# jaesung-cs/vulkan_radix_sort

Measured on AMD Instinct MI355X. Metric: GItems/s at N=2^25 (keys & key+value); achieved HBM GB/s vs peak, higher is better.
Workload: dtype u32

## Files before the change

vulkan_radix_sort_amd/csrc/vrdx_kernels.hip:

```cpp
#include <hip/hip_runtime.h>
#include <stdint.h>

#include <type_traits>

#include "vrdx_kernels.h"
#include "vrdx_layout.h"

namespace vrdx {



#ifdef VRDX_TRACE
#define VRDX_STAMP(slot)                                      \
  do {                                                        \
    if (a.trace != nullptr && tid == 0) stamps[slot] = wall_clock64(); \
  } while (0)
#else
#define VRDX_STAMP(slot) \
  do {                   \
  } while (0)
#endif


typedef uint32_t u32x4 __attribute__((ext_vector_type(4)));
// ... 1992 lines not shown
    lo += v[k] & 0xFFFFu;
    hi += v[k] >> 16;
  }
  if (tid < 64u) {
    const uint32_t mine = tid < 2 * WORDS ? total[tid] : 0u;
    const uint32_t inclusive = WaveInclusiveScan(mine);
    if (tid < 2 * WORDS) {
      uint32_t base = inclusive - mine;
#pragma unroll
      for (uint32_t q = 0; q < 16; ++q) base += below[q];
      a.bucketBase[firstBucket + tid] = base;
      if (topWindow) a.bucketCount[firstBucket + tid] = mine;
      if (mine > a.cap) atomicOr(a.overflowWord, kMsdDeclineBucket);
    }
  }
}

template <uint32_t BITS, bool KV>
__device__ __forceinline__ void ScatterMsdBody(const MsdArgs a) {
  constexpr int THREADS = 1024, KPT = 32, WAVES = THREADS / 64;
  constexpr uint32_t TILE = kMsdTileKeys, D = 1u << BITS, ROW = D / 2u;
  static_assert(THREADS * KPT == TILE && ROW <= (uint32_t)THREADS && WAVES * ROW <= TILE, "geometry");
  extern __shared__ __attribute__((aligned(16))) uint32_t smem[];
  uint32_t* const sorted = smem;
  uint32_t* const counters = smem;
  uint32_t* const tileOffset = smem + TILE;
  uint32_t* const scanScratch = tileOffset + D;

  const int tid = threadIdx.x;
  const int lane = tid & 63;
  const int wave = tid >> 6;
  const uint32_t n = ElementCount(a.maxCount, a.countPtr);
  const uint32_t perXcd = gridDim.x / 8u;
  const uint32_t tile = (blockIdx.x % 8u) * perXcd + blockIdx.x / 8u;
  const uint32_t slots = a.tileKeys / (uint32_t)THREADS;
  const uint32_t frame = a.tileKeys;
  const uint32_t tileStart = tile * frame;
  const uint32_t decided = *a.overflowWord;
  if ((decided & kMsdDeclineMask) != 0u) {
    if (blockIdx.x == 0 && tid == 0 && a.declinedPlans != nullptr) atomicAdd(a.declinedPlans, 1u);
    return;
  }
  const uint32_t SHIFT = (decided >> kMsdShiftShift) & kMsdShiftMask;
  if (((decided >> kMsdModeShift) & kMsdModeMask) == kMsdModeIdentical) {
    if (blockIdx.x == 0 && tid == 0) *a.planWord = kMsdVerdictSorted;
    return;
  }
  const uint32_t valid = tile < a.tiles && tileStart < n ? ((n - tileStart) < frame ? (n - tileStart) : frame) : 0u;
  const uint32_t tileEnd = tileStart + valid;
  const uint32_t loadBase = tileStart + wave * (slots * 64) + lane;
  uint32_t key[KPT];
  LoadStriped<KPT, true, true>(a.keysCaller, loadBase, tileEnd, valid == frame, 0xFFFFFFFFu, key, slots);
  uint32_t prefixWord = 0, base0 = 0, base1 = 0;
  if ((uint32_t)tid < ROW && valid != 0) {
    prefixWord = a.tileCounts[(size_t)tile * ROW + tid];
    base0 = a.bucketBase[2 * tid];
    base1 = a.bucketBase[2 * tid + 1];
  }
  if (blockIdx.x == 0 && tid == 0) *a.planWord = kMsdVerdictRuns | (SHIFT << kMsdShiftShift);
  if (valid == 0) return;

  uint32_t* const myRow = counters + wave * ROW;
#pragma unroll
  for (uint32_t i = 0; i < ROW / 256u; ++i) reinterpret_cast<u32x4*>(myRow)[lane + 64 * i] = u32x4{0u, 0u, 0u, 0u};
  uint32_t rank[KPT / 2];
  RankPacked16<KPT, true>(key, SHIFT, BITS, myRow, lane, rank, slots);
  ForgetDerivedValues<KPT>(key);
  LdsBarrier();

  uint32_t column[WAVES];
  const uint32_t totals = (uint32_t)tid < ROW ? ColumnRead<ROW, WAVES>(counters, tid, column) : 0u;
  const uint32_t count0 = totals & 0xFFFFu, count1 = totals >> 16;
  const uint32_t local0 = BlockExclusiveScanAll<THREADS>(count0 + count1, scanScratch, tid);
  const uint32_t local1 = local0 + count0;
  if ((uint32_t)tid < ROW) {
    ColumnBasesFrom<ROW, WAVES>(counters, tid, local0 | (local1 << 16), column);
    tileOffset[2 * tid] = base0 + (prefixWord & 0xFFFFu) - local0;
    tileOffset[2 * tid + 1] = base1 + (prefixWord >> 16) - local1;
  }
  LdsBarrier();
  PositionsPacked16<KPT, TILE, true>(key, SHIFT, BITS, myRow, rank, slots);
  LdsBarrier();
#pragma unroll
  for (int i = 0; i < KPT; ++i) {
    if (i % 4 == 0 && (uint32_t)i >= slots) break;
    sorted[(rank[i / 2] >> (16 * (i % 2))) & 0xFFFFu] = key[i];
  }
  LdsBarrier();
  uint32_t val[KV ? KPT : 1];
  if constexpr (KV)
    LoadStriped<KPT, true, true>(a.valuesCaller, loadBase, tileEnd, valid == frame, 0u, val, slots);

  constexpr int QUADS = KPT / 4;
  constexpr int B = 4;
  uint32_t quadDigits[KV ? QUADS : 1];
  uint32_t boundaryQuad[2] = {~0u, ~0u};
  uint32_t boundaryDigits[2][2] = {{0, 0}, {0, 0}};
  if ((uint32_t)tid < ROW) {
    if (count0 != 0 && (local0 & 3u) != 0 && local0 < valid) boundaryQuad[0] = local0 & ~3u;
    if (count1 != 0 && (local1 & 3u) != 0 && local1 < valid) boundaryQuad[1] = local1 & ~3u;
  }
  if (tid == 0 && (valid & 3u) != 0) boundaryQuad[0] = valid & ~3u;
  auto scatterQuads = [&](uint32_t* out, bool keysPhase) {
#pragma unroll
    for (int j0 = 0; j0 < QUADS; j0 += B) {
      if (4u * (uint32_t)j0 * THREADS >= valid) break;
      u32x4 w4[B];
      uint32_t o[B];
      bool whole[B];
#pragma unroll
      for (int b = 0; b < B; ++b) w4[b] = *reinterpret_cast<const u32x4*>(&sorted[4u * (tid + (j0 + b) * THREADS)]);
#pragma unroll
      for (int b = 0; b < B; ++b) {
        const int j = j0 + b;
        const uint32_t p = StagingSlot<TILE>(4u * (tid + j * THREADS));
        uint32_t d0, d3;
        if (keysPhase) {
          d0 = __builtin_amdgcn_ubfe(w4[b][0], SHIFT, BITS);
          d3 = __builtin_amdgcn_ubfe(w4[b][3], SHIFT, BITS);
          if constexpr (KV) quadDigits[j] = d0 | (d3 << 16);
        } else {
          d0 = quadDigits[KV ? j : 0] & 0xFFFFu;
          d3 = quadDigits[KV ? j : 0] >> 16;
        }
        whole[b] = p + 3 < valid && d0 == d3;
        o[b] = tileOffset[d0] + p;
        asm volatile("" : "+v"(o[b]));
      }
#pragma unroll
      for (int b = 0; b < B; ++b)
        if (whole[b]) StoreQuad(out, o[b], w4[b]);
    }
#pragma unroll
    for (int s = 0; s < 2; ++s) {
      if (boundaryQuad[s] == ~0u) continue;
      const u32x4 q = *reinterpret_cast<const u32x4*>(&sorted[StagingSlot<TILE>(boundaryQuad[s])]);
      if (keysPhase) {
        boundaryDigits[s][0] = __builtin_amdgcn_ubfe(q[0], SHIFT, BITS) | (__builtin_amdgcn_ubfe(q[1], SHIFT, BITS) << 16);
        boundaryDigits[s][1] = __builtin_amdgcn_ubfe(q[2], SHIFT, BITS) | (__builtin_amdgcn_ubfe(q[3], SHIFT, BITS) << 16);
      }
#pragma unroll
      for (int c = 0; c < 4; ++c) {
        const uint32_t d = (boundaryDigits[s][c / 2] >> (16 * (c % 2))) & 0xFFFFu;
        if (boundaryQuad[s] + c < valid) StoreWord(out, tileOffset[d] + boundaryQuad[s] + c, q[c]);
      }
    }
  };
  scatterQuads(a.keysScratch, true);
  if constexpr (KV) {
    LdsBarrier();
#pragma unroll
    for (int i = 0; i < KPT; ++i) {
      if (i % 4 == 0 && (uint32_t)i >= slots) break;
      sorted[(rank[i / 2] >> (16 * (i % 2))) & 0xFFFFu] = val[i];
    }
    LdsBarrier();
    scatterQuads(a.valuesScratch, false);
  }
}

template <uint32_t BITS>
__device__ __forceinline__ void ScatterMsdPairBody(const MsdArgs a) {
  constexpr int THREADS = 1024, KPT = 32, WAVES = THREADS / 64;
  constexpr uint32_t TILE = kMsdTileKeys, D = 1u << BITS, ROW = D / 2u;
  static_assert(2 * WAVES * ROW <= TILE, "both sub-tiles' counter rows inside the staging buffer");
  extern __shared__ __attribute__((aligned(16))) uint32_t smem[];
  uint32_t* const sorted = smem;
  uint32_t* const counters = smem;
  uint32_t* const tileOffset = smem + TILE;
  uint32_t* const scanScratch = tileOffset + D;

  const int tid = threadIdx.x;
  const int lane = tid & 63;
  const int wave = tid >> 6;
  const uint32_t n = ElementCount(a.maxCount, a.countPtr);
  const uint32_t pairs = (a.tiles + 1u) / 2u;
  const uint32_t perXcd = (pairs + 7u) / 8u;
  const uint32_t pair = (blockIdx.x % 8u) * perXcd + blockIdx.x / 8u;
  const uint32_t slots = a.tileKeys / (uint32_t)THREADS;
  const uint32_t frame = a.tileKeys;
  const uint32_t decided = *a.overflowWord;
  if ((decided & kMsdDeclineMask) != 0u) {
    if (blockIdx.x == 0 && tid == 0 && a.declinedPlans != nullptr) atomicAdd(a.declinedPlans, 1u);
    return;
  }
  const uint32_t SHIFT = (decided >> kMsdShiftShift) & kMsdShiftMask;
  if (((decided >> kMsdModeShift) & kMsdModeMask) == kMsdModeIdentical) {
    if (blockIdx.x == 0 && tid == 0) *a.planWord = kMsdVerdictSorted;
    return;
  }
  const uint32_t tileA = 2u * pair;
  const uint32_t startA = tileA * frame, startB = startA + frame;
  const bool exists = blockIdx.x < 8u * perXcd && pair < pairs && startA < n;
  const uint32_t left = exists ? n - startA : 0u;
  const uint32_t validA = left < frame ? left : frame;
  const uint32_t validB = left > frame ? (left - frame < frame ? left - frame : frame) : 0u;
  const uint32_t valid = validA + validB;
  const uint32_t baseA = startA + wave * (slots * 64) + lane, baseB = baseA + frame;
  uint32_t keyA[KPT], keyB[KPT];
  LoadStriped<KPT, true, true>(a.keysCaller, baseA, startA + validA, validA == frame, 0xFFFFFFFFu, keyA, slots);
  LoadStriped<KPT, true, true>(a.keysCaller, baseB, startB + validB, validB == frame, 0xFFFFFFFFu, keyB, slots);
  uint32_t prefixWord = 0, base0 = 0, base1 = 0;
  if ((uint32_t)tid < ROW && valid != 0) {
    prefixWord = a.tileCounts[(size_t)tileA * ROW + tid];
    base0 = a.bucketBase[2 * tid];
    base1 = a.bucketBase[2 * tid + 1];
  }
  if (blockIdx.x == 0 && tid == 0) *a.planWord = kMsdVerdictRuns | (SHIFT << kMsdShiftShift);
  if (valid == 0) return;

  uint32_t* const rowA = counters + wave * ROW;
  uint32_t* const rowB = counters + (WAVES + wave) * ROW;
#pragma unroll
  for (uint32_t i = 0; i < ROW / 256u; ++i) {
    reinterpret_cast<u32x4*>(rowA)[lane + 64 * i] = u32x4{0u, 0u, 0u, 0u};
    reinterpret_cast<u32x4*>(rowB)[lane + 64 * i] = u32x4{0u, 0u, 0u, 0u};
  }
  uint32_t posA[KPT / 2], posB[KPT / 2];
  RankPacked16<KPT, true>(keyA, SHIFT, BITS, rowA, lane, posA, slots);
  ForgetDerivedValues<KPT>(keyA);
  RankPacked16<KPT, true>(keyB, SHIFT, BITS, rowB, lane, posB, slots);
  ForgetDerivedValues<KPT>(keyB);
  LdsBarrier();

  const uint32_t totals = (uint32_t)tid < ROW ? ColumnTotals<ROW, 2 * WAVES>(counters, tid) : 0u;
  const uint32_t count0 = totals & 0xFFFFu, count1 = totals >> 16;
  const uint32_t local0 = BlockExclusiveScanAll<THREADS>(count0 + count1, scanScratch, tid);
  const uint32_t local1 = local0 + count0;
  if ((uint32_t)tid < ROW) {
    ColumnBases<ROW, 2 * WAVES>(counters, tid, local0 | (local1 << 16));
    tileOffset[2 * tid] = base0 + (prefixWord & 0xFFFFu) - local0;
    tileOffset[2 * tid + 1] = base1 + (prefixWord >> 16) - local1;
  }
  LdsBarrier();
  PositionsPacked16<KPT, TILE, true, true>(keyA, SHIFT, BITS, rowA, posA, slots);
  PositionsPacked16<KPT, TILE, true, true>(keyB, SHIFT, BITS, rowB, posB, slots);
  LdsBarrier();

  constexpr int QUADS = KPT / 4;
  constexpr int B = 2;
  uint32_t boundaryQuad[2] = {~0u, ~0u};
  if ((uint32_t)tid < ROW) {
    if (count0 != 0 && (local0 & 3u) != 0 && local0 < valid) boundaryQuad[0] = local0 & ~3u;
    if (count1 != 0 && (local1 & 3u) != 0 && local1 < valid) boundaryQuad[1] = local1 & ~3u;
  }
  if (tid == 0 && (valid & 3u) != 0) boundaryQuad[0] = valid & ~3u;
#pragma unroll 1
  for (uint32_t half = 0; half < 2; ++half) {
    const uint32_t from = half * frame;
    if (from >= valid) break;
    if (half != 0) LdsBarrier();
#pragma unroll
    for (int i = 0; i < KPT; ++i) {
      if (i % 4 == 0 && (uint32_t)i >= slots) break;
      const uint32_t pa = ((posA[i / 2] >> (16 * (i % 2))) & 0xFFFFu) - from;
      const uint32_t pb = ((posB[i / 2] >> (16 * (i % 2))) & 0xFFFFu) - from;
      if (pa < frame) sorted[StagingSlot<TILE>(pa)] = keyA[i];
      if (pb < frame) sorted[StagingSlot<TILE>(pb)] = keyB[i];
    }
    LdsBarrier();
    const uint32_t here = valid - from < frame ? valid - from : frame;
#pragma unroll
    for (int j0 = 0; j0 < QUADS; j0 += B) {
      if (4u * (uint32_t)j0 * THREADS >= here) break;
      u32x4 w4[B];
      uint32_t o[B];
      bool whole[B];
#pragma unroll
      for (int b = 0; b < B; ++b) w4[b] = *reinterpret_cast<const u32x4*>(&sorted[4u * (tid + (j0 + b) * THREADS)]);
#pragma unroll
      for (int b = 0; b < B; ++b) {
        const uint32_t p = StagingSlot<TILE>(4u * (tid + (j0 + b) * THREADS));
        const uint32_t d0 = __builtin_amdgcn_ubfe(w4[b][0], SHIFT, BITS), d3 = __builtin_amdgcn_ubfe(w4[b][3], SHIFT, BITS);
        whole[b] = p + 3 < here && d0 == d3;
        o[b] = tileOffset[d0] + from + p;
        asm volatile("" : "+v"(o[b]));
      }
#pragma unroll
      for (int b = 0; b < B; ++b)
        if (whole[b]) StoreQuad(a.keysScratch, o[b], w4[b]);
    }
#pragma unroll
    for (int s = 0; s < 2; ++s) {
      const uint32_t q0 = boundaryQuad[s] - from;
      if (boundaryQuad[s] == ~0u || q0 >= frame) continue;
      const u32x4 q = *reinterpret_cast<const u32x4*>(&sorted[StagingSlot<TILE>(q0)]);
#pragma unroll
      for (int c = 0; c < 4; ++c)
        if (q0 + c < here) StoreWord(a.keysScratch, tileOffset[__builtin_amdgcn_ubfe(q[c], SHIFT, BITS)] + boundaryQuad[s] + c, q[c]);
    }
  }
}
template <uint32_t BITS, bool KV>
constexpr bool MsdScatterTakesPairs() { return !KV && BITS == 10; }
template <uint32_t BITS, bool KV>
__device__ __forceinline__ void ScatterMsdRole(const MsdArgs a) {
  if constexpr (MsdScatterTakesPairs<BITS, KV>())
    ScatterMsdPairBody<BITS>(a);
  else
    ScatterMsdBody<BITS, KV>(a);
}


template <uint32_t BITS, int KPT, bool KV, int THREADS = 1024>
__device__ __forceinline__ void BucketSort2Bucket(const MsdArgs a, const uint32_t bucket, const uint32_t below, const bool streamOut) {
  constexpr int WAVES = THREADS / 64;
  static_assert(THREADS == 1024 || THREADS == 512, "one or two words of a counter row per thread");
  constexpr uint32_t TILE = THREADS * KPT;
  constexpr uint32_t ROW = 1024;
  static_assert(32u - BITS <= 22u, "two passes of at most eleven bits");
  static_assert(TILE <= 65536 && WAVES * ROW <= TILE && KPT % 4 == 0, "packed positions; the staging buffer covers the counters");
  extern __shared__ __attribute__((aligned(16))) uint32_t smem[];
  uint32_t* const staged = smem;
  uint32_t* const counters = smem;
  uint32_t* const scanScratch = smem + TILE;

  const int tid = threadIdx.x;
  const int lane = tid & 63;
  const int wave = tid >> 6;
  const uint32_t W0 = (below + 1u) / 2u, W1 = below / 2u;
  constexpr uint32_t passes = 2u;
  const uint32_t myBase = (uint32_t)__builtin_amdgcn_readfirstlane((int)a.bucketBase[bucket]);
  const uint32_t n = (uint32_t)__builtin_amdgcn_readfirstlane((int)a.bucketCount[bucket]);
  if (n == 0) return;
  const uint32_t* const keysIn = a.keysScratch + myBase;
  uint32_t* const keysOut = a.keysCaller + myBase;
  const uint32_t* const valuesIn = KV ? a.valuesScratch + myBase : nullptr;
  uint32_t* const valuesOut = KV ? a.valuesCaller + myBase : nullptr;

  constexpr bool DYN = true;
  const uint32_t chunks = (n + 255u) / 256u;
  const uint32_t base = chunks / WAVES, extra = chunks % WAVES;
  const uint32_t w = (uint32_t)__builtin_amdgcn_readfirstlane(wave);
  const uint32_t slots = 4u * (base + (w < extra ? 1u : 0u));
  const uint32_t first = 256u * (w * base + (w < extra ? w : extra)) + lane;
  uint32_t key[KPT];
  uint32_t val[KV ? KPT : 1];
  LoadStriped<KPT, false, DYN>(keysIn, first, n, false, 0xFFFFFFFFu, key, slots);
  if constexpr (KV) LoadStriped<KPT, false, DYN>(valuesIn, first, n, false, 0u, val, slots);

  uint32_t* const myRow = counters + wave * ROW;
#pragma unroll 1
  for (uint32_t pass = 0; pass < passes; ++pass) {
    const uint32_t shift = pass == 0 ? 0u : W0;
    const uint32_t width = pass == 0 ? W0 : W1;
    const uint32_t words = width > 1u ? 1u << (width - 1u) : 1u;
#pragma unroll
    for (uint32_t i = 0; i < ROW / 256u; ++i)
      if (256u * i < words) reinterpret_cast<u32x4*>(myRow)[lane + 64 * i] = u32x4{0u, 0u, 0u, 0u};
    uint32_t rank[KPT / 2];
    RankPacked16<KPT, DYN>(key, shift, width, myRow, lane, rank, slots);
    ForgetDerivedValues<KPT>(key);
    LdsBarrier();
    uint32_t firstNow = first;
    asm volatile("" : "+v"(firstNow));
    if constexpr (THREADS == 512) {
      const bool mine = KV || 2u * (uint32_t)tid < words;
      u32x2 column[WAVES];
      const u32x2 totals = mine ? ColumnPairRead<ROW, WAVES>(counters, tid, column) : u32x2{0u, 0u};
      const uint32_t count0 = totals[0] & 0xFFFFu, count1 = totals[0] >> 16, count2 = totals[1] & 0xFFFFu;
      const uint32_t local0 = BlockExclusiveScanAll<THREADS>(count0 + count1 + count2 + (totals[1] >> 16), scanScratch + 16 * pass, tid);
      const uint32_t local2 = local0 + count0 + count1;
      if (mine)
        ColumnPairBasesFrom<ROW, WAVES>(counters, tid, u32x2{local0 | ((local0 + count0) << 16), local2 | ((local2 + count2) << 16)}, column);
    } else if constexpr (!KV) {
      const bool mine = (uint32_t)tid < words;
      uint32_t column[WAVES];
      const uint32_t totals = mine ? ColumnRead<ROW, WAVES>(counters, tid, column) : 0u;
      const uint32_t count0 = totals & 0xFFFFu;
      const uint32_t local0 = BlockExclusiveScanAll<THREADS>(count0 + (totals >> 16), scanScratch + 16 * pass, tid);
      if (mine) ColumnBasesFrom<ROW, WAVES>(counters, tid, local0 | ((local0 + count0) << 16), column);
    } else {
      const bool mine = (uint32_t)tid < words;
      const uint32_t totals = mine ? ColumnTotals<ROW, WAVES>(counters, tid) : 0u;
      const uint32_t count0 = totals & 0xFFFFu;
      const uint32_t local0 = BlockExclusiveScanAll<THREADS>(count0 + (totals >> 16), scanScratch + 16 * pass, tid);
      if (mine) ColumnBases<ROW, WAVES>(counters, tid, local0 | ((local0 + count0) << 16));
    }
    LdsBarrier();
    PositionsPacked16<KPT, TILE, DYN>(key, shift, width, myRow, rank, slots);
    LdsBarrier();
#pragma unroll
    for (int i = 0; i < KPT; ++i) {
      if (DYN && i % 4 == 0 && (uint32_t)i >= slots) break;
      staged[(rank[i / 2] >> (16 * (i % 2))) & 0xFFFFu] = key[i];
    }
    LdsBarrier();
#pragma unroll
    for (int i = 0; i < KPT; ++i) {
      if (DYN && i % 4 == 0 && (uint32_t)i >= slots) break;
      key[i] = staged[StagingSlot<TILE>(firstNow + 64 * i)];
    }
    if constexpr (KV) {
      LdsBarrier();
#pragma unroll
      for (int i = 0; i < KPT; ++i) {
        if (DYN && i % 4 == 0 && (uint32_t)i >= slots) break;
        staged[(rank[i / 2] >> (16 * (i % 2))) & 0xFFFFu] = val[i];
      }
      LdsBarrier();
#pragma unroll
      for (int i = 0; i < KPT; ++i) {
        if (DYN && i % 4 == 0 && (uint32_t)i >= slots) break;
        val[i] = staged[StagingSlot<TILE>(firstNow + 64 * i)];
      }
    }
    LdsBarrier();
  }
  if (KV ? a.maxCount > kStreamingLoadsAbove : streamOut) {
    asm volatile("; non-temporal output" ::: "memory");
#pragma unroll
    for (int i = 0; i < KPT; ++i) {
      if (DYN && i % 4 == 0 && (uint32_t)i >= slots) break;
      const uint32_t index = first + 64 * i;
      if (index < n) {
        __builtin_nontemporal_store(key[i], &keysOut[index]);
        if constexpr (KV) __builtin_nontemporal_store(val[i], &valuesOut[index]);
      }
    }
    asm volatile("" ::: "memory");
  } else {
#pragma unroll
    for (int i = 0; i < KPT; ++i) {
      if (DYN && i % 4 == 0 && (uint32_t)i >= slots) break;
      const uint32_t index = first + 64 * i;
      if (index < n) {
        keysOut[index] = key[i];
        if constexpr (KV) valuesOut[index] = val[i];
      }
    }
  }
}

template <uint32_t BITS, int KPT, bool KV, int THREADS = 1024>
__device__ __forceinline__ void BucketSort2Body(const MsdArgs a, const uint32_t workgroups) {
  const uint32_t verdict = *a.planWord;
  if ((verdict & kMsdVerdictMask) != kMsdVerdictRuns) return;
  const uint32_t below = (verdict >> kMsdShiftShift) & kMsdShiftMask;
  uint32_t streamedBuckets = 0u;
  if constexpr (!KV && THREADS == 1024 && BITS == 10)
    if (a.maxCount > kStreamingLoadsAbove) streamedBuckets = (1u << BITS) - min(a.plainTail, 1u << BITS);
#pragma unroll 1
  for (uint32_t bucket = blockIdx.x; bucket < (1u << BITS); bucket += workgroups)
    BucketSort2Bucket<BITS, KPT, KV, THREADS>(a, bucket, below, bucket < streamedBuckets);
}

template <uint32_t BITS, bool KV>
__global__ __launch_bounds__(512, 4) void bucket_sort2_half_kernel(MsdArgs a) {
  BucketSort2Body<BITS, kMsdHalfCap / 512, KV, 512>(a, gridDim.x);
}

template <uint32_t BITS, bool KV, bool DYN>
__device__ __forceinline__ void FallbackPassBody(const OnesweepArgs p) {
  if constexpr (KV)
    OnesweepBody<1024, 32, true, true, DYN>(p);
  else
    OnesweepPairBody<1024, 32, DYN>(p);
}

template <uint32_t BITS, bool KV, bool DYN>
__global__ __launch_bounds__(1024) void msd_scatter_or_pass0_kernel(MsdArgs m, OnesweepArgs p) {
  if ((*m.overflowWord & kMsdDeclineMask) == 0u) {
    ScatterMsdRole<BITS, KV>(m);
    return;
  }
  if (blockIdx.x > p.statusRows) return;
  FallbackPassBody<BITS, KV, DYN>(p);
  if (blockIdx.x == 0 && threadIdx.x == 0 && m.declinedPlans != nullptr) atomicAdd(m.declinedPlans, 1u);
}
template <uint32_t BITS, bool KV, bool DYN>
__global__ __launch_bounds__(1024) void msd_buckets_or_pass1_kernel(MsdArgs m, OnesweepArgs p) {
  const uint32_t verdict = *m.planWord & kMsdVerdictMask;
  if (verdict < kMsdVerdictRuns) {
    if (blockIdx.x > p.statusRows) return;
    FallbackPassBody<BITS, KV, DYN>(p);
    return;
  }
  const uint32_t workgroups = min(gridDim.x, (1u << BITS) / 2u);
  if (verdict == kMsdVerdictRuns && blockIdx.x < workgroups)
    BucketSort2Body<BITS, (KV ? kMsdCapKeyValue : kMsdCapKeys) / 1024, KV>(m, workgroups);
}

__device__ __forceinline__ uint32_t OrderCheckKey(uint32_t tid, uint32_t wave, uint32_t slot) {
  uint32_t x = (blockIdx.x * 1024u + tid) * 0x9E3779B9u + slot * 0x85EBCA6Bu;
  x ^= x >> 15; x *= 0x2C1B3C6Du; x ^= x >> 12; x *= 0x297A2D39u; x ^= x >> 15;
  const uint32_t mode = (blockIdx.x + wave + slot) % 6u;
  const uint32_t mask = mode == 0 ? 0u : mode == 1 ? 1u : mode == 2 ? 3u : mode == 3 ? 15u : mode == 4 ? 0x21u : 255u;
  return x & mask;
}

__global__ __launch_bounds__(1024) void lds_order_check_kernel(uint32_t* mismatches, uint32_t* sticky) {
  __shared__ uint32_t counters[2 * 16 * 256];
  const int tid = threadIdx.x, lane = tid & 63, wave = tid >> 6;
  for (int i = tid; i < 2 * 16 * 256; i += 1024) counters[i] = 0;
  __syncthreads();
  uint32_t* const histA = counters + wave * 256;
  uint32_t* const histB = counters + (16 + wave) * 256;
  uint32_t bad = 0;
  for (uint32_t round = 0; round < 8; ++round) {
    uint32_t key[8], ra[8], rb[8];
#pragma unroll
    for (int i = 0; i < 8; ++i) key[i] = OrderCheckKey(tid, wave, round * 8 + i);
    RankAtomic<8, false>(key, 0, histA, lane, ra);
    RankBallot<8>(key, 0, histB, lane, rb);
#pragma unroll
    for (int i = 0; i < 8; ++i) bad += ra[i] != rb[i];
  }
#pragma unroll 1
  for (uint32_t form = 0; form < 2; ++form) {
    uint32_t key[32], want[16];
#pragma unroll
    for (int i = 0; i < 32; ++i) key[i] = OrderCheckKey(tid, wave, 64 + 32 * form + i);
    RankBallot<32, true>(key, 0, histB, lane, want);
    if (form == 0) {
      uint32_t ra[32];
      RankAtomic<32, false>(key, 0, histA, lane, ra);
#pragma unroll
      for (int i = 0; i < 16; ++i) bad += (ra[2 * i] | (ra[2 * i + 1] << 16)) != want[i];
    } else {
      uint32_t rp[16];
      RankAtomic<32, true>(key, 0, histA, lane, rp);
#pragma unroll
      for (int i = 0; i < 16; ++i) bad += rp[i] != want[i];
    }
  }
  if (bad != 0) {
    if (mismatches != nullptr) atomicAdd(mismatches, bad);
    if (sticky != nullptr) atomicOr(sticky, 2u);
  }
}

__device__ __forceinline__ uint32_t OrderCheckDigit11(uint32_t tid, uint32_t wave, uint32_t slot) {
  uint32_t x = (blockIdx.x * 1024u + tid) * 0x9E3779B9u + slot * 0x85EBCA6Bu + 0x7F4A7C15u;
  x ^= x >> 15; x *= 0x2C1B3C6Du; x ^= x >> 12; x *= 0x297A2D39u; x ^= x >> 15;
  const uint32_t mode = (blockIdx.x + wave + slot) % 7u;
  const uint32_t mask = mode == 0 ? 0u : mode == 1 ? 1u : mode == 2 ? 3u : mode == 3 ? 15u : mode == 4 ? 0x421u : mode == 5 ? 63u : 2047u;
  return ((x & mask) + (mode == 5 ? 0x300u : 0u)) & 2047u;
}

__global__ __launch_bounds__(1024) void lds_order_check_packed_kernel(uint32_t* mismatches, uint32_t* sticky) {
  extern __shared__ __attribute__((aligned(16))) uint32_t smem[];
  const int tid = threadIdx.x, lane = tid & 63, wave = tid >> 6;
  uint32_t* const rowA = smem + wave * 1024;
  uint32_t* const rowB = smem + (16 + wave) * 1024;
  for (int i = lane; i < 1024; i += 64) rowA[i] = rowB[i] = 0;
  uint32_t bad = 0;
#pragma unroll 1
  for (uint32_t round = 0; round < 4; ++round) {
    uint32_t key[16], got[8];
#pragma unroll
    for (int i = 0; i < 16; ++i) key[i] = OrderCheckDigit11(tid, wave, round * 16 + i);
    RankPacked16<16, false>(key, 0, 11u, rowA, lane, got);
#pragma unroll
    for (int i = 0; i < 16; ++i) {
      const uint32_t d = key[i];
      uint64_t same = ~0ull;
#pragma unroll
      for (int b = 0; b < 11; ++b) {
        const bool bit = (d >> b) & 1u;
        const uint64_t ballot = __ballot(bit);
        same &= bit ? ballot : ~ballot;
      }
      const uint32_t below = LanesBelow(same);
      const uint32_t sh = (d & 1u) * 16u;
      const uint32_t prior = (__hip_atomic_load(&rowB[d >> 1], __ATOMIC_RELAXED, __HIP_MEMORY_SCOPE_WORKGROUP) >> sh) & 0xFFFFu;
      if (below == 0)
        (void)__hip_atomic_fetch_add(&rowB[d >> 1], (uint32_t)__popcll(same) << sh, __ATOMIC_RELAXED, __HIP_MEMORY_SCOPE_WORKGROUP);
      bad += ((got[i / 2] >> (16 * (i % 2))) & 0xFFFFu) != prior + below;
    }
  }
  if (bad != 0) {
    if (mismatches != nullptr) atomicAdd(mismatches, bad);
    if (sticky != nullptr) atomicOr(sticky, 2u);
  }
}

__global__ __launch_bounds__(64) void spin_kernel(unsigned long long* out, uint32_t ticks) {
  const unsigned long long t0 = wall_clock64();
  unsigned long long t = t0;
  while (t - t0 < ticks) {
    __builtin_amdgcn_s_sleep(1);
    t = wall_clock64();
  }
  if (threadIdx.x == 0) {
    out[0] = t0;
    out[1] = t;
  }
}

typedef u32x4 u32x4_a8 __attribute__((aligned(8)));

__device__ __forceinline__ uint32_t Sort64First(uint32_t n, bool* whole) {
  const uint32_t i = (blockIdx.x * kSort64Threads + threadIdx.x) * 4u;
  *whole = i + 4u <= n;
  return i;
}

template <bool IOTA>
__global__ __launch_bounds__(kSort64Threads) void split64_kernel(const uint64_t* __restrict__ keys, uint32_t* __restrict__ lo,
                                                                 uint32_t* __restrict__ other, uint32_t n) {
  bool whole;
  const uint32_t i = Sort64First(n, &whole);
  if (i >= n) return;
  if (whole) {
    const u32x4_a8* const pairs = reinterpret_cast<const u32x4_a8*>(keys + i);
    const u32x4 a = pairs[0], b = pairs[1];
    *reinterpret_cast<u32x4*>(lo + i) = u32x4{a.x, a.z, b.x, b.z};
    *reinterpret_cast<u32x4*>(other + i) = IOTA ? u32x4{i, i + 1u, i + 2u, i + 3u} : u32x4{a.y, a.w, b.y, b.w};
    return;
  }
  for (uint32_t j = i; j < n; ++j) {
    const uint64_t k = keys[j];
    lo[j] = (uint32_t)k;
    other[j] = IOTA ? j : (uint32_t)(k >> 32);
  }
}

__global__ __launch_bounds__(kSort64Threads) void merge64_kernel(uint64_t* __restrict__ keys, const uint32_t* __restrict__ lo,
                                                                 const uint32_t* __restrict__ hi, uint32_t n) {
  bool whole;
  const uint32_t i = Sort64First(n, &whole);
  if (i >= n) return;
  if (whole) {
    const u32x4 l = *reinterpret_cast<const u32x4*>(lo + i), h = *reinterpret_cast<const u32x4*>(hi + i);
    u32x4_a8* const pairs = reinterpret_cast<u32x4_a8*>(keys + i);
    pairs[0] = u32x4{l.x, h.x, l.y, h.y};
    pairs[1] = u32x4{l.z, h.z, l.w, h.w};
    return;
  }
  for (uint32_t j = i; j < n; ++j) keys[j] = (uint64_t)hi[j] << 32 | lo[j];
}

__global__ __launch_bounds__(kSort64Threads) void gather_hi64_kernel(const uint64_t* __restrict__ keys,
                                                                     const uint32_t* __restrict__ index,
                                                                     uint32_t* __restrict__ hi, uint32_t n) {
  bool whole;
  const uint32_t i = Sort64First(n, &whole);
  if (i >= n) return;
  const uint32_t* const words = reinterpret_cast<const uint32_t*>(keys);
  if (whole) {
    const u32x4 at = *reinterpret_cast<const u32x4*>(index + i);
    *reinterpret_cast<u32x4*>(hi + i) = u32x4{words[2ull * at.x + 1u], words[2ull * at.y + 1u], words[2ull * at.z + 1u],
                                              words[2ull * at.w + 1u]};
    return;
  }
  for (uint32_t j = i; j < n; ++j) hi[j] = words[2ull * index[j] + 1u];
}

__global__ __launch_bounds__(kSort64Threads) void permute64_kernel(const uint64_t* __restrict__ keys,
                                                                   const uint32_t* __restrict__ values,
                                                                   const uint32_t* __restrict__ index,
                                                                   uint32_t* __restrict__ hiThenValues,
                                                                   uint64_t* __restrict__ keysOut, uint32_t n) {
  bool whole;
  const uint32_t i = Sort64First(n, &whole);
  if (i >= n) return;
  const uint32_t* const words = reinterpret_cast<const uint32_t*>(keys);
  if (whole) {
    const u32x4 at = *reinterpret_cast<const u32x4*>(index + i);
    const u32x4 h = *reinterpret_cast<const u32x4*>(hiThenValues + i);
    const u32x4 l = u32x4{words[2ull * at.x], words[2ull * at.y], words[2ull * at.z], words[2ull * at.w]};
    const u32x4 v = u32x4{values[at.x], values[at.y], values[at.z], values[at.w]};
    u32x4* const pairs = reinterpret_cast<u32x4*>(keysOut + i);
    pairs[0] = u32x4{l.x, h.x, l.y, h.y};
    pairs[1] = u32x4{l.z, h.z, l.w, h.w};
    *reinterpret_cast<u32x4*>(hiThenValues + i) = v;
    return;
  }
  for (uint32_t j = i; j < n; ++j) {
    const uint32_t at = index[j];
    keysOut[j] = (uint64_t)hiThenValues[j] << 32 | words[2ull * at];
    hiThenValues[j] = values[at];
  }
}

__global__ __launch_bounds__(kSort64Threads) void copy_back64_kernel(uint64_t* __restrict__ keys, uint32_t* __restrict__ values,
                                                                     const uint64_t* __restrict__ keysIn,
                                                                     const uint32_t* __restrict__ valuesIn, uint32_t n) {
  bool whole;
  const uint32_t i = Sort64First(n, &whole);
  if (i >= n) return;
  if (whole) {
    const u32x4* const in = reinterpret_cast<const u32x4*>(keysIn + i);
    const u32x4 a = in[0], b = in[1], v = *reinterpret_cast<const u32x4*>(valuesIn + i);
    u32x4_a8* const pairs = reinterpret_cast<u32x4_a8*>(keys + i);
    pairs[0] = a;
    pairs[1] = b;
    *reinterpret_cast<u32x4_a4*>(values + i) = v;
    return;
  }
  for (uint32_t j = i; j < n; ++j) {
    keys[j] = keysIn[j];
    values[j] = valuesIn[j];
  }
}


#include "vrdx_launch.inc"

static const void* const kStubs[kNumKernels] = {
#define VRDX_KERNEL_STUB(id, stub, threads, ldsBytes, name) reinterpret_cast<const void*>(stub),
    VRDX_KERNELS(VRDX_KERNEL_STUB)
#undef VRDX_KERNEL_STUB
};

static hipError_t PrepareKernel(KernelId id) {
  const uint32_t lds = kKernelShapes[id].ldsBytes;
  if (lds == 0) return hipSuccess;
  return hipFuncSetAttribute(kStubs[id], hipFuncAttributeMaxDynamicSharedMemorySize, (int)lds);
}

static hipError_t LaunchKernel(KernelId id, uint32_t grid, hipStream_t stream, void** params) {
  const KernelShape& k = kKernelShapes[id];
  return hipLaunchKernel(kStubs[id], dim3(grid), dim3(k.threads), params, k.ldsBytes, stream);
}

}
```

Before: 147.9.

## Vectorize keys-only bucket sort loads and store final tile straight from LDS

For keys-only bucket sorting, keys are now loaded as 16-byte quads per lane instead of striped scalar loads. The pad value is derived from the bucket's prefix so padded slots sort last. On the final pass the kernel skips reading scattered keys back into registers and writes the LDS staging buffer out with vectorized, coalesced quad stores, with a scalar tail fix-up. This cuts load and store instruction counts and one LDS round trip. It adds unaligned-quad access and tail-handling complexity.

```diff
diff --git a/vulkan_radix_sort_amd/csrc/vrdx_kernels.hip b/vulkan_radix_sort_amd/csrc/vrdx_kernels.hip
--- a/vulkan_radix_sort_amd/csrc/vrdx_kernels.hip
+++ b/vulkan_radix_sort_amd/csrc/vrdx_kernels.hip
@@ -2318,6 +2318,76 @@
 }
 
 
+template <int KPT>
+__device__ __forceinline__ void LoadChunkQuads(const uint32_t* base, uint32_t first4, uint32_t n, uint32_t pad,
+                                               uint32_t (&out)[KPT], uint32_t slots) {
+  static_assert(KPT % 4 == 0, "whole chunks");
+  const char* const bytes = reinterpret_cast<const char*>(base);
+  const uint32_t offset = first4 * 4u;
+  StaticFor<0, KPT, 4>([&](auto slot) {
+    constexpr int i = decltype(slot)::value;
+    if ((uint32_t)i >= slots) return false;
+    const uint32_t element = first4 + 64 * i;
+    const char* const p = bytes + ((uint64_t)offset + (uint64_t)(i * 256));
+    u32x4 q = {pad, pad, pad, pad};
+    if (element + 3 < n) {
+      q = *reinterpret_cast<const u32x4_a4*>(p);
+    } else {
+#pragma unroll
+      for (int c = 0; c < 3; ++c)
+        if (element + c < n) q[c] = reinterpret_cast<const uint32_t*>(p)[c];
+    }
+#pragma unroll
+    for (int c = 0; c < 4; ++c) out[i + c] = q[c];
+    return true;
+  });
+}
+
+template <uint32_t TILE, int THREADS, int KPT, bool NT>
+__device__ __forceinline__ void StoreStagedBucket(const uint32_t* staged, uint32_t* out, uint32_t n, int tid) {
+  static_assert((4u * THREADS) % 2048u == 0, "StagingSlot(4 tid + 4 THREADS j) = StagingSlot(4 tid) + 4 THREADS j");
+  const uint32_t mine = 4u * (uint32_t)tid;
+  const uint32_t slot = StagingSlot<TILE>(mine);
+  StaticFor<0, KPT / 4, 1>([&](auto quad) {
+    constexpr int j = decltype(quad)::value;
+    if (4u * (uint32_t)j * THREADS >= n) return false;
+    const u32x4 q = *reinterpret_cast<const u32x4*>(&staged[slot + 4u * j * THREADS]);
+    char* const rowBytes = reinterpret_cast<char*>(out + 4u * j * THREADS);
+    u32x4_a4* const to = reinterpret_cast<u32x4_a4*>(rowBytes + (uint64_t)(mine * 4u));
+    if (mine + 4u * j * THREADS + 3u < n) {
+      if constexpr (NT)
+        __builtin_nontemporal_store(q, to);
+      else
+        *to = q;
+    }
+    return true;
+  });
+  if ((n & 3u) != 0 && (uint32_t)tid == (n >> 2) % THREADS) {
+    const uint32_t p = n & ~3u;
+    const u32x4 q = *reinterpret_cast<const u32x4*>(&staged[StagingSlot<TILE>(p)]);
+#pragma unroll
+    for (int c = 0; c < 3; ++c) {
+      if (p + c < n) {
+        if constexpr (NT)
+          __builtin_nontemporal_store(q[c], &out[p + c]);
+        else
+          out[p + c] = q[c];
+      }
+    }
+  }
+}
+
+template <uint32_t TILE, int THREADS, int KPT>
+__device__ __forceinline__ void StoreStagedBucketAs(const uint32_t* staged, uint32_t* out, uint32_t n, int tid, bool streaming) {
+  if (streaming) {
+    asm volatile("; non-temporal output" ::: "memory");
+    StoreStagedBucket<TILE, THREADS, KPT, true>(staged, out, n, tid);
+    asm volatile("" ::: "memory");
+  } else {
+    StoreStagedBucket<TILE, THREADS, KPT, false>(staged, out, n, tid);
+  }
+}
+
 template <uint32_t BITS, int KPT, bool KV, int THREADS = 1024>
 __device__ __forceinline__ void BucketSort2Bucket(const MsdArgs a, const uint32_t bucket, const uint32_t below, const bool streamOut) {
   constexpr int WAVES = THREADS / 64;
@@ -2352,8 +2422,13 @@
   const uint32_t first = 256u * (w * base + (w < extra ? w : extra)) + lane;
   uint32_t key[KPT];
   uint32_t val[KV ? KPT : 1];
-  LoadStriped<KPT, false, DYN>(keysIn, first, n, false, 0xFFFFFFFFu, key, slots);
-  if constexpr (KV) LoadStriped<KPT, false, DYN>(valuesIn, first, n, false, 0u, val, slots);
+  if constexpr (KV) {
+    LoadStriped<KPT, false, DYN>(keysIn, first, n, false, 0xFFFFFFFFu, key, slots);
+    LoadStriped<KPT, false, DYN>(valuesIn, first, n, false, 0u, val, slots);
+  } else {
+    const uint32_t pad = keysIn[0] | ((1u << below) - 1u);
+    LoadChunkQuads<KPT>(keysIn, first - lane + 4u * lane, n, pad, key, slots);
+  }
 
   uint32_t* const myRow = counters + wave * ROW;
 #pragma unroll 1
@@ -2402,6 +2477,8 @@
       staged[(rank[i / 2] >> (16 * (i % 2))) & 0xFFFFu] = key[i];
     }
     LdsBarrier();
+    if constexpr (!KV)
+      if (pass + 1u == passes) break;
 #pragma unroll
     for (int i = 0; i < KPT; ++i) {
       if (DYN && i % 4 == 0 && (uint32_t)i >= slots) break;
@@ -2423,7 +2500,10 @@
     }
     LdsBarrier();
   }
-  if (KV ? a.maxCount > kStreamingLoadsAbove : streamOut) {
+  if constexpr (!KV) {
+    StoreStagedBucketAs<TILE, THREADS, KPT>(staged, keysOut, n, tid, streamOut);
+    LdsBarrier();
+  } else if (a.maxCount > kStreamingLoadsAbove) {
     asm volatile("; non-temporal output" ::: "memory");
 #pragma unroll
     for (int i = 0; i < KPT; ++i) {
@@ -2431,7 +2511,7 @@
       const uint32_t index = first + 64 * i;
       if (index < n) {
         __builtin_nontemporal_store(key[i], &keysOut[index]);
-        if constexpr (KV) __builtin_nontemporal_store(val[i], &valuesOut[index]);
+        __builtin_nontemporal_store(val[i], &valuesOut[index]);
       }
     }
     asm volatile("" ::: "memory");
@@ -2442,7 +2522,7 @@
       const uint32_t index = first + 64 * i;
       if (index < n) {
         keysOut[index] = key[i];
-        if constexpr (KV) valuesOut[index] = val[i];
+        valuesOut[index] = val[i];
       }
     }
   }
```

After: 152.2, median of 6. 1.03x the previous value.
